# jd-opensource/xllm-service

Measured on NVIDIA H100. Metric: requests/sec tokenize+hash+match @4K-token prompts, higher is better.
Workload: dtype u64

## Files before the change

### xllm_service_b200/csrc/common.cuh

```cuda
#pragma once
#include <cuda_runtime.h>
#include <stdint.h>
#include <stdio.h>

#include <mutex>

#define XLLM_OK 0
#define XLLM_ERR_INVALID_ARG (-1)
#define XLLM_ERR_CUDA (-2)
#define XLLM_ERR_IO (-3)
#define XLLM_ERR_FORMAT (-4)
#define XLLM_ERR_UNSUPPORTED (-5)
#define XLLM_ERR_CAPACITY (-6)
#define XLLM_ERR_NOMEM (-7)

namespace xllm {

void set_last_error(const char* fmt, ...);

#define XLLM_CUDA_TRY(expr)                                                              \
  do {                                                                                   \
    cudaError_t _e = (expr);                                                             \
    if (_e != cudaSuccess) {                                                             \
      ::xllm::set_last_error("%s:%d: %s -> %s", __FILE__, __LINE__, #expr,               \
                             cudaGetErrorString(_e));                                    \
      return XLLM_ERR_CUDA;                                                              \
    }                                                                                    \
  } while (0)

#define XLLM_TRY_RC(expr)          \
  do {                             \
    const int _rc = (expr);        \
    if (_rc != XLLM_OK) return _rc; \
  } while (0)

__device__ __forceinline__ uint32_t smem_u32(const void* p) {
  return static_cast<uint32_t>(__cvta_generic_to_shared(p));
}

__device__ __forceinline__ void cp_async_16(void* smem_dst, const void* gmem_src) {
  asm volatile("cp.async.cg.shared.global [%0], [%1], 16;\n" ::"r"(smem_u32(smem_dst)), "l"(gmem_src)
               : "memory");
}
__device__ __forceinline__ void cp_async_4(void* smem_dst, const void* gmem_src) {
  asm volatile("cp.async.ca.shared.global [%0], [%1], 4;\n" ::"r"(smem_u32(smem_dst)), "l"(gmem_src)
               : "memory");
}
__device__ __forceinline__ void cp_async_commit() { asm volatile("cp.async.commit_group;\n" ::: "memory"); }
template <int N>
__device__ __forceinline__ void cp_async_wait() {
  asm volatile("cp.async.wait_group %0;\n" ::"n"(N) : "memory");
}

struct DeviceOnce {
  static constexpr int kMaxDevices = 64;
  std::once_flag flag[kMaxDevices];
  int n_sm[kMaxDevices] = {0};
  cudaError_t err[kMaxDevices] = {cudaSuccess};
  template <typename F>
  int get(F&& setup, cudaError_t* e, int* device = nullptr) {
    int dev = 0;
    *e = cudaGetDevice(&dev);
    if (*e != cudaSuccess) return 0;
    if (device) *device = dev;
    if (dev < 0 || dev >= kMaxDevices) { *e = cudaErrorInvalidDevice; return 0; }
    std::call_once(flag[dev], [&] {
      int n = 0;
      cudaError_t r = cudaDeviceGetAttribute(&n, cudaDevAttrMultiProcessorCount, dev);
      if (r == cudaSuccess) r = setup();
      n_sm[dev] = n;
      err[dev] = r;
    });
    *e = err[dev];
    return *e == cudaSuccess ? n_sm[dev] : 0;
  }
};

}
```

### xllm_service_b200/csrc/sp_encode.cu

```cuda
#include "sp_encode.cuh"

#include <stdlib.h>
#include <string.h>

#include <type_traits>
#include <vector>

#include "common.cuh"
#include "sp_long_word.cuh"

namespace xllm {

namespace {

constexpr int kNBuf = 2048;
constexpr int kFastWin = 128;
constexpr int kExpWin = 512;
constexpr int kPrefetchFirst = 2;
constexpr int kPrefetchWindows = 2;
constexpr int kLongEnterAt = 1024;
constexpr int kLongFlushAt = 1024;
constexpr int kMaxSym = 16;
constexpr int kCoopMaxSym = 512;
constexpr int kMaxWords = 704;
constexpr uint32_t kFull = 0xffffffffu;
constexpr size_t kWarmSliceBytes = (size_t)kNBuf * 4 + (size_t)kMaxWords * 2;
constexpr uint16_t kNotPre = 0xFFFFu;
constexpr uint32_t kResolvedFlag = 0x40000000u;

template <bool SMALL>
struct PMOps;
template <>
struct PMOps<false> {
  using T = uint2;
  static constexpr uint32_t kNone = kNoPrio;
  static __device__ __forceinline__ T pack(uint2 v) { return v; }
  static __device__ __forceinline__ T none() { return make_uint2(kNoPrio, 0); }
  static __device__ __forceinline__ uint32_t prio(T v) { return v.x; }
  static __device__ __forceinline__ uint32_t merged(T v) { return v.y; }
  static __device__ __forceinline__ uint32_t prio_at(const T* p) { return p->x; }
};
template <>
struct PMOps<true> {
  using T = uint32_t;
  static constexpr uint32_t kNone = 0xFFFFu;
  static __device__ __forceinline__ T pack(uint2 v) { return v.x == kNoPrio ? 0xFFFF0000u : ((v.x << 16) | v.y); }
  static __device__ __forceinline__ T none() { return 0xFFFF0000u; }
  static __device__ __forceinline__ uint32_t prio(T v) { return v >> 16; }
  static __device__ __forceinline__ uint32_t merged(T v) { return v & 0xFFFFu; }
  static __device__ __forceinline__ uint32_t prio_at(const T* p) {
    return reinterpret_cast<const uint16_t*>(p)[1];
  }
};

constexpr int kHfRows = 32;
template <bool SMALL, int ROWS = kMaxSym>
struct WarpSmemT {
  static constexpr int kRows = ROWS;
  static constexpr int kSyms = ROWS * 32 > kCoopMaxSym ? ROWS * 32 : kCoopMaxSym;
  uint32_t S[kSyms];
  typename PMOps<SMALL>::T PM[kSyms];
  uint8_t nbuf[kNBuf];
  uint16_t wstart[kMaxWords];
  uint16_t pend[32];
};
constexpr int kUniMaxMatch = 32;
template <bool SMALL>
struct WarpSmemUniT : WarpSmemT<SMALL> {
  uint32_t mlist[32 * kUniMaxMatch];
};

__device__ __forceinline__ uint32_t hash_pair(uint32_t a, uint32_t b) {
  return (a * 0x9E3779B1u + b) * 0x85EBCA6Bu;
}
__device__ __forceinline__ uint32_t hash_cp(uint32_t cp) {
  uint32_t h = cp * 0x9E3779B1u;
  h ^= h >> 16;
  return h;
}

struct PairProbe {
  uint32_t h;
  uint4 e;
};
__device__ __forceinline__ PairProbe pair_probe_begin(const SpDev& T, uint32_t a, uint32_t b) {
  PairProbe p;
  p.h = hash_pair(a, b) >> T.pair_shift;
  p.e = ((a | b) & kSymUnknownFlag) ? make_uint4(kEmptyKey, 0, 0, 0)
                                    : __ldg(reinterpret_cast<const uint4*>(T.pair_table) + p.h);
  return p;
}
__device__ __forceinline__ uint2 pair_probe_finish(const SpDev& T, uint32_t a, uint32_t b, PairProbe p) {
  for (;;) {
    if (p.e.x == a && p.e.y == b) return make_uint2(p.e.z, p.e.w);
    if (p.e.x == kEmptyKey) return make_uint2(kNoPrio, 0);
    p.h = (p.h + 1) & T.pair_mask;
    p.e = __ldg(reinterpret_cast<const uint4*>(T.pair_table) + p.h);
  }
}
__device__ __forceinline__ uint2 pair_lookup(const SpDev& T, uint32_t a, uint32_t b) {
  return pair_probe_finish(T, a, b, pair_probe_begin(T, a, b));
}

__device__ __forceinline__ uint32_t cp_lookup(const SpDev& T, uint32_t cp) {
  if (cp == 0x2581u) return T.space_sym;
  uint32_t h = hash_cp(cp) & T.cp_mask;
  for (;;) {
    const uint2 e = __ldg(reinterpret_cast<const uint2*>(T.cp_table) + h);
    if (e.x == cp) return e.y;
    if (e.x == kEmptyKey) return kSymUnknownFlag | cp;
    h = (h + 1) & T.cp_mask;
  }
}

__device__ __forceinline__ uint32_t utf8_unit(const uint8_t* p, uint32_t avail, uint8_t b0, bool* valid) {
  *valid = true;
  if (b0 < 0x80) return 1;
  auto trail = [](uint8_t x) { return (x & 0xC0) == 0x80; };
  if (avail >= 2 && (b0 & 0xE0) == 0xC0) {
    const uint8_t b1 = p[1];
    const uint32_t cp = ((b0 & 0x1Fu) << 6) | (b1 & 0x3Fu);
    if (trail(b1) && cp >= 0x80) return 2;
  } else if (avail >= 3 && (b0 & 0xF0) == 0xE0) {
    const uint8_t b1 = p[1], b2 = p[2];
    const uint32_t cp = ((b0 & 0x0Fu) << 12) | ((b1 & 0x3Fu) << 6) | (b2 & 0x3Fu);
    if (trail(b1) && trail(b2) && cp >= 0x800 && !(cp >= 0xD800 && cp < 0xE000)) return 3;
  } else if (avail >= 4 && (b0 & 0xF8) == 0xF0) {
    const uint8_t b1 = p[1], b2 = p[2], b3 = p[3];
    const uint32_t cp = ((b0 & 0x07u) << 18) | ((b1 & 0x3Fu) << 12) | ((b2 & 0x3Fu) << 6) | (b3 & 0x3Fu);
    if (trail(b1) && trail(b2) && trail(b3) && cp >= 0x10000 && cp <= 0x10FFFF) return 4;
  }
  *valid = false;
  return 1;
}

__device__ __forceinline__ uint32_t char_sym(const SpDev& T, const uint8_t* p, uint32_t* adv) {
  const uint32_t b0 = p[0];
  if (b0 < 0x80 || T.byte_mode) {
    *adv = 1;
    return __ldg(T.ascii_sym + b0);
  }
  uint32_t cp, l;
  if (b0 < 0xE0) { l = 2; cp = ((b0 & 0x1F) << 6) | (p[1] & 0x3F); }
  else if (b0 < 0xF0) { l = 3; cp = ((b0 & 0x0F) << 12) | ((p[1] & 0x3Fu) << 6) | (p[2] & 0x3F); }
  else { l = 4; cp = ((b0 & 0x07) << 18) | ((p[1] & 0x3Fu) << 12) | ((p[2] & 0x3Fu) << 6) | (p[3] & 0x3F); }
  *adv = l;
  return cp_lookup(T, cp);
}

__device__ __forceinline__ int sym_ids(const SpDev& T, uint32_t sym, int32_t out[4], bool* unk) {
  uint32_t cp;
  *unk = false;
  if (!(sym & kSymUnknownFlag)) {
    const int32_t e = __ldg(T.emit + sym);
    if (e >= 0) { out[0] = e; return 1; }
    if (e == -2) return 0;
    cp = __ldg(T.virt_cp + (sym - T.n_pieces));
  } else {
    cp = sym & 0x1FFFFFu;
  }
  *unk = true;
  if (!T.byte_fallback) { out[0] = T.unk_id; return 1; }
  uint8_t b[4];
  int n;
  if (cp < 0x80) { b[0] = (uint8_t)cp; n = 1; }
  else if (cp < 0x800) { b[0] = 0xC0 | (cp >> 6); b[1] = 0x80 | (cp & 0x3F); n = 2; }
  else if (cp < 0x10000) { b[0] = 0xE0 | (cp >> 12); b[1] = 0x80 | ((cp >> 6) & 0x3F); b[2] = 0x80 | (cp & 0x3F); n = 3; }
  else { b[0] = 0xF0 | (cp >> 18); b[1] = 0x80 | ((cp >> 12) & 0x3F); b[2] = 0x80 | ((cp >> 6) & 0x3F); b[3] = 0x80 | (cp & 0x3F); n = 4; }
  for (int i = 0; i < n; ++i) out[i] = __ldg(T.byte_id + b[i]);
  return n;
// ... 672 lines not shown
__device__ int unigram_backtrack(SM& sm, const uint8_t* w, int len, int lane);
template <typename SM>
__device__ int unigram_word_slow(const SpDev& T, SM& sm, const uint8_t* w, int len, float* score, int lane);

template <typename SM>
__device__ int unigram_word(const SpDev& T, SM& sm, const uint8_t* w, int len, float* score, int lane) {
  float* best = reinterpret_cast<float*>(sm.S);
  uint32_t* back = reinterpret_cast<uint32_t*>(sm.PM);
  for (int e = lane; e <= len; e += 32) back[e] = 0;
  if (lane == 0) best[0] = *score;
  __syncwarp();
  for (int s0 = 0; s0 < len; s0 += 32) {
    const int s = s0 + lane;
    const bool is_start = s < len && (w[s] & 0xC0) != 0x80;
    int cnt = 0;
    bool overflow = false;
    if (is_start) {
      const uint8_t b0 = w[s];
      int clen = b0 < 0x80 ? 1 : (b0 < 0xE0 ? 2 : (b0 < 0xF0 ? 3 : 4));
      if (clen > len - s) clen = len - s;
      const int max_l = (int)T.max_piece_len < len - s ? (int)T.max_piece_len : len - s;
      uint32_t node = 0;
      bool has_single = false;
      for (int L = 1; L <= max_l; ++L) {
        int32_t piece;
        if (!uni_trie_step(T, node, w[s + L - 1], &node, &piece)) break;
        if (piece >= 0) {
          if (cnt < kUniMaxMatch) sm.mlist[lane * kUniMaxMatch + cnt] = ((uint32_t)L << 24) | (uint32_t)piece;
          else overflow = true;
          ++cnt;
          has_single |= L == clen;
        }
      }
      if (!has_single) {
        if (cnt < kUniMaxMatch) sm.mlist[lane * kUniMaxMatch + cnt] = ((uint32_t)clen << 24) | 0xFFFFFFu;
        else overflow = true;
        ++cnt;
      }
    }
    if (__any_sync(kFull, overflow)) return unigram_word_slow(T, sm, w, len, score, lane);
    __syncwarp();
    uint32_t starts = __ballot_sync(kFull, is_start);
    while (starts) {
      const int b = __ffs(starts) - 1;
      starts &= starts - 1;
      const int sb = s0 + b;
      const int nb_ = __shfl_sync(kFull, cnt, b);
      const float base = best[sb];
      if (lane < nb_) {
        const uint32_t m = sm.mlist[b * kUniMaxMatch + lane];
        const int L = (int)(m >> 24);
        const uint32_t id = m & 0xFFFFFFu;
        const int e = sb + L;
        const double cand = id == 0xFFFFFFu ? (double)(T.unk_score + base)
                                            : (double)__ldg(T.piece_score + id) + (double)base;
        if (back[e] == 0 || cand > (double)best[e]) {
          best[e] = (float)cand;
          back[e] = m;
        }
      }
      __syncwarp();
    }
  }
  const float end_score = best[len];
  __syncwarp();
  const int n = unigram_backtrack(sm, w, len, lane);
  *score = end_score;
  __syncwarp();
  return n;
}

template <typename SM>
__device__ int unigram_backtrack(SM& sm, const uint8_t* w, int len, int lane) {
  const uint32_t* back = reinterpret_cast<const uint32_t*>(sm.PM);
  int n = 0;
  for (int e = len; e > 0; e -= (int)(back[e] >> 24)) ++n;
  __syncwarp();
  if (lane == 0) {
    int k = n;
    for (int e = len; e > 0;) {
      const uint32_t link = back[e];
      const int L = (int)(link >> 24);
      uint32_t sym;
      if ((link & 0xFFFFFFu) != 0xFFFFFFu) {
        sym = kResolvedFlag | (link & 0xFFFFFFu);
      } else {
        const uint8_t* p = w + e - L;
        const uint32_t b0 = p[0];
        uint32_t cp = b0;
        if (L == 2) cp = ((b0 & 0x1F) << 6) | (p[1] & 0x3F);
        else if (L == 3) cp = ((b0 & 0x0F) << 12) | ((p[1] & 0x3Fu) << 6) | (p[2] & 0x3F);
        else if (L == 4) cp = ((b0 & 0x07) << 18) | ((p[1] & 0x3Fu) << 12) | ((p[2] & 0x3Fu) << 6) | (p[3] & 0x3F);
        sym = kSymUnknownFlag | cp;
      }
      sm.S[--k] = sym;
      e -= L;
    }
  }
  __syncwarp();
  return n;
}

template <typename SM>
__device__ int unigram_word_slow(const SpDev& T, SM& sm, const uint8_t* w, int len, float* score, int lane) {
  float* best = reinterpret_cast<float*>(sm.S);
  uint32_t* back = reinterpret_cast<uint32_t*>(sm.PM);
  static_assert(sizeof(sm.S) >= 4 * (kUniMaxWord + 1) && sizeof(sm.PM) >= 4 * (kUniMaxWord + 1), "lattice scratch");
  if (lane == 0) best[0] = *score;
  __syncwarp();
  const int passes = ((int)T.max_piece_len + 31) / 32;
  for (int e = 1; e <= len; ++e) {
    if (e < len && (w[e] & 0xC0) == 0x80) continue;
    int cs = e - 1;
    while (cs > 0 && (w[cs] & 0xC0) == 0x80) --cs;
    const int clen = e - cs;
    float best_f = 0.f;
    uint32_t best_link = 0;
    bool first = true;
    for (int pass = passes - 1; pass >= 0; --pass) {
      const int L = pass * 32 + lane + 1;
      const int s = e - L;
      int32_t id = -1;
      if (L <= (int)T.max_piece_len && s >= 0 && (w[s] & 0xC0) != 0x80) id = hf_vocab_lookup(T, w + s, L);
      const bool unk = id < 0 && L == clen;
      double cand = 0.0;
      if (id >= 0) cand = (double)__ldg(T.piece_score + id) + (double)best[s];
      else if (unk) cand = (double)(T.unk_score + best[s]);
      uint32_t m = __ballot_sync(kFull, id >= 0 || unk);
      while (m) {
        const int src = 31 - __clz(m);
        m &= ~(1u << src);
        const double c = __shfl_sync(kFull, cand, src);
        const int32_t cid = __shfl_sync(kFull, id, src);
        if (first || c > (double)best_f) {
          best_f = (float)c;
          best_link = ((uint32_t)(pass * 32 + src + 1) << 24) | (cid >= 0 ? (uint32_t)cid : 0xFFFFFFu);
          first = false;
        }
      }
    }
    if (lane == 0) { best[e] = best_f; back[e] = best_link; }
    __syncwarp();
  }
  const float end_score = best[len];
  __syncwarp();
  const int n = unigram_backtrack(sm, w, len, lane);
  *score = end_score;
  __syncwarp();
  return n;
}

#ifdef XLLM_EXP_STATS
constexpr int kExpStats = 32;
enum : int { kExpStatTimed = 16, kExpStatCycWindow = 17, kExpStatCycProbe = 18, kExpStatCycEmit = 19 };
__device__ unsigned long long g_exp_stats[kExpStats];
#define EXP_STAT(i) do { if (lane == 0) atomicAdd(&g_exp_stats[i], 1ull); } while (0)
#define EXP_CLOCK(t) (t = clock64())
#else
#define EXP_STAT(i) do { } while (0)
#define EXP_CLOCK(t) do { } while (0)
#endif

struct ExpReq {
  const uint8_t* src;
  uint32_t len;
  int32_t* out;
  int64_t cap;
  int64_t n_out;
  bool P;
  bool S;
  bool U;
};
constexpr int kExpWords = 64;
template <bool SMALL>
struct ExpSmemT {
  uint32_t S[kMaxSym * 32];
  typename PMOps<SMALL>::T PM[kMaxSym * 32];
  uint4 txt[kExpWin / 16 + 1];
  uint16_t ex[2 * (kExpWords + 2)];
};
constexpr int kExpLongWords = 4;
constexpr int kExpLongEvery = 512;
struct ExpResume {
  uint32_t pos;
  uint32_t flags;
  long long n_out;
};

struct ExpLongWord {
  uint32_t end;
  int32_t n_out;
  bool done;
  bool unk;
};

template <bool SMALL, typename SM>
__device__ __noinline__ ExpLongWord express_long_word(const SpDev& T, SM& sm, const uint32_t* base, uint32_t nwords,
                                                      uint32_t vlen, uint32_t v0, bool lead, int32_t* out, int32_t cap,
                                                      int32_t n_out, bool prev_unk, int lane) {
  const ExpLongWord not_done{0u, n_out, false, prev_unk};
  uint32_t end = 0;
  bool found = false;
  for (uint32_t wb = v0 & ~3u; !found; wb += (uint32_t)kFastWin) {
    if (wb - (v0 & ~3u) > (uint32_t)kCoopMaxSym) return not_done;
    const uint32_t i = (wb >> 2) + (uint32_t)lane;
    uint32_t w = i < nwords ? __ldg(base + i) : 0x20202020u;
    const uint32_t b0 = wb + 4u * lane;
    uint32_t sp4 = 0, bad4 = 0;
#pragma unroll
    for (int k = 0; k < 4; ++k) {
      const uint32_t bk = (w >> (8 * k)) & 0xFFu;
      const uint32_t at = b0 + k;
      if (at < v0) continue;
      if (at >= vlen) { sp4 |= 1u << k; continue; }
      if (bk >= 0x80u) { bad4 |= 1u << k; continue; }
      const bool spl = bk == 0x20u || ((T.spacelike_ascii[(bk >> 5) & 3] >> (bk & 31)) & 1u);
      const bool simple = (T.simple_ascii[(bk >> 5) & 3] >> (bk & 31)) & 1u;
      if (spl && (bk != 0x20u || simple)) sp4 |= 1u << k;
      else if (!simple) bad4 |= 1u << k;
    }
    const uint32_t spm = __ballot_sync(kFull, sp4 != 0u), badm = __ballot_sync(kFull, bad4 != 0u);
    if (spm) {
      const int L = __ffs(spm) - 1;
      const uint32_t sL = __shfl_sync(kFull, sp4, L), bL = __shfl_sync(kFull, bad4, L);
      const int k = __ffs(sL) - 1;
      if ((badm & ((1u << L) - 1u)) || (bL & ((1u << k) - 1u))) return not_done;
      end = wb + 4u * L + k;
      found = true;
    } else if (badm) {
      return not_done;
    }
  }
  const int nbytes = (int)(end - v0);
  const int nsym = nbytes + (lead ? 1 : 0);
  if (nbytes < 1 || nsym > kCoopMaxSym) return not_done;
  const uint8_t* bytes = reinterpret_cast<const uint8_t*>(base) + v0;
  __syncwarp();
  if (lead && lane == 0) sm.S[0] = T.space_sym;
  for (int i = lane; i < nbytes; i += 32) sm.S[i + (lead ? 1 : 0)] = __ldg(T.ascii_sym + __ldg(bytes + i));
  __syncwarp();
  const int n = coop_merge<SMALL>(T, sm, nsym, lane);
  for (int b = 0; b < n; b += 32) {
    const int j = b + lane;
    int32_t tmp[4];
    bool unk = false;
    int c = 0;
    if (j < n) c = sym_ids(T, sm.S[j], tmp, &unk);
    if (!T.byte_fallback) {
      const uint32_t um = __ballot_sync(kFull, j < n && unk);
      const bool prev = lane == 0 ? prev_unk : ((um >> (lane - 1)) & 1u);
      if (unk && prev) c = 0;
      const int lastl = (n - b) >= 32 ? 31 : (n - b - 1);
      prev_unk = (um >> lastl) & 1u;
    }
    const int inc = warp_incl_scan(c, lane);
    int32_t o = n_out + (inc - c);
    for (int k = 0; k < c; ++k, ++o)
      if (o < cap) out[o] = tmp[k];
    n_out += __shfl_sync(kFull, inc, 31);
  }
  if (T.byte_fallback) prev_unk = false;
  __syncwarp();
  return ExpLongWord{end, n_out, true, prev_unk};
}

__device__ __forceinline__ uint32_t exp_blank(uint32_t x, int i, int lo, int hi) {
  const int a = min(max(lo - 4 * i, 0), 4), b = min(max(hi - 4 * i, 0), 4);
  const uint32_t below_b = b >= 4 ? 0xFFFFFFFFu : (1u << (8 * b)) - 1u, below_a = a >= 4 ? 0xFFFFFFFFu : (1u << (8 * a)) - 1u;
  const uint32_t keep = below_b & ~below_a;
  return (x & keep) | (0x20202020u & ~keep);
}
__device__ __forceinline__ uint32_t exp_space4(uint32_t x) {
  x ^= 0x20202020u;
  const uint32_t z = ~(((x & 0x7F7F7F7Fu) + 0x7F7F7F7Fu) | x | 0x7F7F7F7Fu);
  return (((z >> 7) * 0x01020408u) >> 24) & 0xFu;
}
__device__ __forceinline__ U128 exp_word_key(const uint4* txt, uint32_t s, int n, bool lead) {
  const uint2* t8 = reinterpret_cast<const uint2*>(txt) + (s >> 3);
  const uint2 u0 = t8[0], u1 = t8[1], u2 = t8[2];
  const bool odd = (s & 4u) != 0u;
  const uint32_t bsh = (s & 3u) * 8u;
  const uint32_t t0 = odd ? u0.y : u0.x, t1 = odd ? u1.x : u0.y, t2 = odd ? u1.y : u1.x, t3 = odd ? u2.x : u1.y,
                 t4 = odd ? u2.y : u2.x;
  unsigned long long lo = (unsigned long long)__funnelshift_r(t0, t1, bsh) | ((unsigned long long)__funnelshift_r(t1, t2, bsh) << 32);
  unsigned long long hi = (unsigned long long)__funnelshift_r(t2, t3, bsh) | ((unsigned long long)__funnelshift_r(t3, t4, bsh) << 32);
  if (n < 8) { lo &= (1ull << (8 * n)) - 1ull; hi = 0ull; }
  else hi &= (1ull << (8 * (n - 8))) - 1ull;
  return U128{(lo << 8) | (unsigned long long)((lead ? 0x80u : 0u) | (uint32_t)n), (hi << 8) | (lo >> 56)};
}
template <bool SMALL>
__device__ __forceinline__ bool exp_probe_finish(MemoRef memo, U128 key, uint32_t slot, U128 k, U128& val) {
  if (k.lo == key.lo && k.hi == key.hi) return MemoIds<SMALL>::valid(val);
  if ((k.lo | k.hi) == 0) return false;
  const uint8_t* e = memo.table + (size_t)(slot ^ 1u) * 32;
  const U128 k2 = ld_b128_cached(e);
  val = ld_b128_cached(e + 16);
  return k2.lo == key.lo && k2.hi == key.hi && MemoIds<SMALL>::valid(val);
}
template <bool SMALL>
__device__ __forceinline__ void exp_store(int32_t* out, U128 val, int cnt, int o, bool c1, bool c2, bool fits,
                                          int32_t cap) {
  if (fits) {
    if (cnt >= 1) out[o] = (int32_t)MemoIds<SMALL>::id(val, 0);
    if (c1 || c2) {
      if (cnt >= 2) out[o + 1] = (int32_t)MemoIds<SMALL>::id(val, 1);
      if (cnt >= 3) out[o + 2] = (int32_t)MemoIds<SMALL>::id(val, 2);
      if (c2) {
#pragma unroll
        for (int q = 3; q < MemoIds<SMALL>::kMax; ++q)
          if (q < cnt) out[o + q] = (int32_t)MemoIds<SMALL>::id(val, q);
      }
    }
  } else {
#pragma unroll
    for (int q = 0; q < MemoIds<SMALL>::kMax; ++q)
      if (q < cnt && o + q < cap) out[o + q] = (int32_t)MemoIds<SMALL>::id(val, q);
  }
}

template <bool SMALL, bool MEMO, typename SM>
__device__ __forceinline__ uint32_t express_run(const SpDev& T, SM& sm, ExpReq& rs, uint32_t pos, int lane,
                                                MemoRef memo, bool* failed) {
  const uint32_t A = (uint32_t)(reinterpret_cast<uintptr_t>(rs.src) & 15u);
  const uint32_t* const base = reinterpret_cast<const uint32_t*>(rs.src - A);
  const uint4* const base16 = reinterpret_cast<const uint4*>(rs.src - A);
  const uint32_t vlen = rs.len + A;
  const uint32_t nwords = (vlen + 3u) >> 2;
  const uint32_t nunits = (vlen + 15u) >> 4;
  bool P = rs.P;
  bool S = rs.S;
  bool U = rs.U;
  int n_long = 0;
  uint16_t* const ex = sm.ex;
  const uint32_t* const ex2 = reinterpret_cast<const uint32_t*>(sm.ex);
  int32_t* const out = rs.out;
  const int32_t cap = rs.cap > 0x7fffffffll ? 0x7fffffff : (int32_t)rs.cap;
  int32_t n_out = (int32_t)rs.n_out;
  const uint32_t lt = (1u << lane) - 1u;
  auto load_window = [&](uint32_t at) {
    const uint32_t i = (at >> 4) + (uint32_t)lane;
    return i < nunits ? __ldg(base16 + i) : make_uint4(0x20202020u, 0x20202020u, 0x20202020u, 0x20202020u);
  };
  uint32_t v = pos + A;
  uint4 w = load_window(v);
  *failed = false;
#ifdef XLLM_EXP_STATS
  unsigned long long t_step = 0, t_vote = 0, t_probe = 0, cyc_window = 0, cyc_probe = 0, cyc_emit = 0, n_timed = 0;
#endif
  for (;;) {
    EXP_CLOCK(t_step);
    const uint32_t skip = v & 15u;
    const uint32_t wb = v - skip;
    const bool at_end = wb + (uint32_t)kExpWin >= vlen;
    if ((skip != 0u && lane == 0) || at_end) {
      const int lo = lane == 0 ? (int)skip : 0;
      const int hi = at_end ? (int)(vlen - wb) - 16 * lane : 16;
      w = make_uint4(exp_blank(w.x, 0, lo, hi), exp_blank(w.y, 1, lo, hi), exp_blank(w.z, 2, lo, hi),
                     exp_blank(w.w, 3, lo, hi));
    }
    {
      bool ok = ((w.x | w.y | w.z | w.w) & 0x80808080u) == 0u;
      bool fast_ok = false;
      if (T.printable_simple)
        fast_ok = (((w.x | 0x80808080u) - 0x20202020u) & ((w.y | 0x80808080u) - 0x20202020u) &
                   ((w.z | 0x80808080u) - 0x20202020u) & ((w.w | 0x80808080u) - 0x20202020u) & 0x80808080u) ==
                      0x80808080u &&
                  (((w.x + 0x01010101u) | (w.y + 0x01010101u) | (w.z + 0x01010101u) | (w.w + 0x01010101u)) &
                   0x80808080u) == 0u;
      if (!__all_sync(kFull, ok && fast_ok)) {
        uint32_t q[4] = {w.x, w.y, w.z, w.w};
#pragma unroll
        for (int k = 0; k < 16; ++k) {
          uint32_t& part = q[k >> 2];
          const uint32_t bk = (part >> (8 * (k & 3))) & 0xFFu;
          const bool spl = (T.spacelike_ascii[(bk >> 5) & 3] >> (bk & 31)) & 1u;
          ok = ok && (spl || ((T.simple_ascii[(bk >> 5) & 3] >> (bk & 31)) & 1u));
          if (spl) part = (part & ~(0xFFu << (8 * (k & 3)))) | (0x20u << (8 * (k & 3)));
        }
        if (!__all_sync(kFull, ok)) { EXP_STAT(4); *failed = true; break; }
        w = make_uint4(q[0], q[1], q[2], q[3]);
      }
    }
    EXP_CLOCK(t_vote);
    const uint32_t ns16 = ~(exp_space4(w.x) | (exp_space4(w.y) << 4) | (exp_space4(w.z) << 8) | (exp_space4(w.w) << 12)) &
                          0xFFFFu;
    sm.txt[lane] = w;
    uint32_t prev_ns = (__shfl_up_sync(kFull, ns16, 1) >> 15) & 1u;
    uint32_t next_ns = __shfl_down_sync(kFull, ns16, 1) & 1u;
    if (lane == 0) prev_ns = 0u;
    if (lane == 31) next_ns = at_end ? 0u : 1u;
    if (!P && !S) {
      if ((__shfl_sync(kFull, ns16, 0) >> skip) & 1u) { EXP_STAT(5); *failed = true; break; }
    }
    const uint32_t st16 = ns16 & ~((ns16 << 1) | prev_ns) & 0xFFFFu;
    const uint32_t en16 = ns16 & ~((ns16 >> 1) | (next_ns << 15)) & 0xFFFFu;
    const uint32_t cs = __popc(st16);
    const uint32_t b0 = __ballot_sync(kFull, cs & 1u), b1 = __ballot_sync(kFull, cs & 2u);
    const uint32_t b2 = __ballot_sync(kFull, cs & 4u), b3 = __ballot_sync(kFull, cs & 8u);
    const uint32_t last_ns = __ballot_sync(kFull, (ns16 & 0x8000u) != 0u) >> 31;
    const int nstart = __popc(b0) + 2 * __popc(b1) + 4 * __popc(b2) + 8 * __popc(b3);
    const int nend = nstart - (int)(at_end ? 0u : last_ns);
    int take = nend < kExpWords ? nend : kExpWords;
    uint32_t cons = at_end ? vlen - wb : (uint32_t)kExpWin - 1u;
    bool S2 = true;
    uint4 w_next = make_uint4(0u, 0u, 0u, 0u);
    auto long_word = [&](uint32_t s0) -> bool {
      ++n_long;
      const bool dense = n_long > kExpLongWords && (uint32_t)n_long * (uint32_t)kExpLongEvery > wb + s0 - A;
      ExpLongWord r{0u, n_out, false, U};
      if (!dense) r = express_long_word<SMALL>(T, sm, base, nwords, vlen, wb + s0, P || (!S && s0 > skip), out, cap,
                                              n_out, U, lane);
      n_out = r.n_out;
      U = r.unk;
      if (!r.done) {
        if (s0 > skip) {
          P = P || !S;
          S = true;
          v = wb + s0;
        }
        *failed = true;
        return false;
      }
      P = false;
      S = false;
      v = r.end;
      if (v >= vlen) return false;
      w = load_window(v);
      return true;
    };
    if (nstart > 0) {
      {
        uint32_t k = __popc(b0 & lt) + 2 * __popc(b1 & lt) + 4 * __popc(b2 & lt) + 8 * __popc(b3 & lt);
        uint32_t e = k - (prev_ns & ns16 & 1u);
        for (uint32_t m = st16; m && k <= (uint32_t)kExpWords; m &= m - 1u, ++k)
          ex[2u * k] = (uint16_t)(16 * lane + __ffs(m) - 1);
        for (uint32_t m = en16; m && e < (uint32_t)kExpWords; m &= m - 1u, ++e)
          ex[2u * e + 1u] = (uint16_t)(16 * lane + __ffs(m) - 1);
      }
      __syncwarp();
      const bool inA = lane < take, inB = lane + 32 < take;
      const uint32_t seA = ex2[inA ? lane : 0], seB = ex2[inB ? lane + 32 : 0];
      const uint32_t sA = seA & 0xFFFFu, sB = seB & 0xFFFFu;
      const int nA = (int)(seA >> 16) - (int)sA + 1, nB = (int)(seB >> 16) - (int)sB + 1;
      const uint32_t lmA = __ballot_sync(kFull, inA && nA > kMemoMaxKeyBytes);
      const uint32_t lmB = __ballot_sync(kFull, inB && nB > kMemoMaxKeyBytes);
      if (lmA) take = __ffs(lmA) - 1;
      else if (lmB) take = 32 + __ffs(lmB) - 1;
      if (take == 0) {
        const uint32_t s0 = ex[0];
        if (!lmA && s0 > skip) {
          cons = s0;
          w_next = load_window(wb + cons);
        } else {
          if (long_word(s0)) { EXP_STAT(6); continue; }
          EXP_STAT(7);
          break;
        }
      } else {
      const bool activeA = lane < take, activeB = lane + 32 < take;
      if (take < nstart) cons = ex[2 * take];
      const bool leadA = lane > 0 || P || (!S && sA > skip);
      const U128 keyA = exp_word_key(sm.txt, sA, nA, leadA), keyB = exp_word_key(sm.txt, sB, nB, true);
      bool hitA = false, hitB = false;
      U128 valA{0ull, 0ull}, valB{0ull, 0ull};
      if constexpr (MEMO) {
        const uint32_t slotA = memo_slot(keyA, memo.mask), slotB = memo_slot(keyB, memo.mask);
        U128 kA{0ull, 0ull}, kB{0ull, 0ull};
        if (activeA) {
          kA = ld_b128_cached(memo.table + (size_t)slotA * 32);
          valA = ld_b128_cached(memo.table + (size_t)slotA * 32 + 16);
        }
        if (activeB) {
          kB = ld_b128_cached(memo.table + (size_t)slotB * 32);
          valB = ld_b128_cached(memo.table + (size_t)slotB * 32 + 16);
        }
        if (activeA) hitA = exp_probe_finish<SMALL>(memo, keyA, slotA, kA, valA);
        if (activeB) hitB = exp_probe_finish<SMALL>(memo, keyB, slotB, kB, valB);
      }
      bool hardA = false, hardB = false;
#pragma unroll 1
      for (int h = 0; h < 2; ++h) {
        if (!(h ? activeB && !hitB : activeA && !hitA)) continue;
        const U128 key = h ? keyB : keyA;
        const unsigned long long lo = (key.lo >> 8) | (key.hi << 56), hi = key.hi >> 8;
        const int n = (int)(key.lo & 0x7Fu);
        int m = 0;
        if (key.lo & 0x80u) { sm.S[lane] = T.space_sym; m = 1; }
        for (int i = 0; i < n; ++i) {
          const uint32_t c = (uint32_t)((i < 8 ? lo >> (8 * i) : hi >> (8 * (i - 8))) & 0xFFull);
          sm.S[(m++) * 32 + lane] = __ldg(T.ascii_sym + c);
        }
        const uint32_t alive = lane_merge<SMALL>(T, sm, m, lane);
        const int k = __popc(alive);
        uint32_t id[8] = {0, 0, 0, 0, 0, 0, 0, 0};
        bool hard = k > MemoIds<SMALL>::kMax;
        int q = 0;
        for (uint32_t mm = alive; mm && !hard; ++q) {
          const int j = __ffs(mm) - 1;
          mm &= mm - 1;
          const uint32_t sym = sm.S[j * 32 + lane];
          int32_t e = -1;
          if (!(sym & kSymUnknownFlag)) e = __ldg(T.emit + sym);
          if (e < 0 || (uint32_t)e >= (SMALL ? (1u << 16) : (1u << 28))) hard = true;
          else id[q] = (uint32_t)e;
        }
        if (!hard) {
          const U128 val = MemoIds<SMALL>::pack(k, id);
          if (h) valB = val;
          else valA = val;
          if constexpr (MEMO) {
            uint32_t slot = memo_slot(key, memo.mask);
            const U128 zero{0ull, 0ull};
#pragma unroll 1
            for (int way = 0; way < 2; ++way, slot ^= 1u) {
              uint8_t* e = memo.table + (size_t)slot * 32;
              const U128 old = cas_b128(e, zero, key);
              if ((old.lo | old.hi) == 0) { st_b128(e + 16, val); break; }
              if (old.lo == key.lo && old.hi == key.hi) break;
            }
          }
        }
        if (h) hardB = hard;
        else hardA = hard;
      }
      {
        const uint32_t hmA = __ballot_sync(kFull, hardA), hmB = __ballot_sync(kFull, hardB);
        EXP_CLOCK(t_probe);
        if (hmA | hmB) {
          const int fh = hmA ? __ffs(hmA) - 1 : 32 + __ffs(hmB) - 1;
          EXP_STAT(8);
          if (fh == 0) {
            if (long_word(ex[0])) continue;
            break;
          }
          take = fh;
          cons = ex[2 * take];
        }
      }
      w_next = load_window(wb + cons);
#ifdef XLLM_EXP_STATS
      { const uint32_t aA = __ballot_sync(kFull, activeA), aB = __ballot_sync(kFull, activeB);
        const uint32_t hA = __ballot_sync(kFull, hitA), hB = __ballot_sync(kFull, hitB);
        if (lane == 0) { atomicAdd(&g_exp_stats[9], (unsigned long long)(__popc(aA) + __popc(aB))); atomicAdd(&g_exp_stats[10], (unsigned long long)(__popc(hA) + __popc(hB))); if ((aA & ~hA) | (aB & ~hB)) atomicAdd(&g_exp_stats[11], 1ull); } }
#endif
      const int cntA = lane < take ? MemoIds<SMALL>::count(valA) : 0;
      const int cntB = lane + 32 < take ? MemoIds<SMALL>::count(valB) : 0;
      const uint32_t a0 = __ballot_sync(kFull, cntA & 1), a1 = __ballot_sync(kFull, cntA & 2), a2 = __ballot_sync(kFull, cntA & 4);
      const uint32_t c0 = __ballot_sync(kFull, cntB & 1), c1 = __ballot_sync(kFull, cntB & 2), c2 = __ballot_sync(kFull, cntB & 4);
      const int totalA = __popc(a0) + 2 * __popc(a1) + 4 * __popc(a2);
      const int totalB = __popc(c0) + 2 * __popc(c1) + 4 * __popc(c2);
      const int oA = n_out + __popc(a0 & lt) + 2 * __popc(a1 & lt) + 4 * __popc(a2 & lt);
      const int oB = n_out + totalA + __popc(c0 & lt) + 2 * __popc(c1 & lt) + 4 * __popc(c2 & lt);
      const bool fits = n_out + totalA + totalB <= cap;
      exp_store<SMALL>(out, valA, cntA, oA, a1 != 0u, a2 != 0u, fits, cap);
      if (c0 | c1 | c2) exp_store<SMALL>(out, valB, cntB, oB, c1 != 0u, c2 != 0u, fits, cap);
      n_out += totalA + totalB;
      U = false;
#ifdef XLLM_EXP_STATS
      { const unsigned long long t = clock64(); cyc_window += t_vote - t_step; cyc_probe += t_probe - t_vote; cyc_emit += t - t_probe; ++n_timed; }
#endif
      if (take == nstart) S2 = !((__shfl_sync(kFull, ns16, (cons - 1u) >> 4) >> ((cons - 1u) & 15u)) & 1u);
      }
    } else {
      w_next = load_window(wb + cons);
    }
    EXP_STAT(1);
    P = S2 && (take > 0 || P || !S);
    S = S2;
    v = wb + cons;
    if (v >= vlen) break;
    w = w_next;
    __syncwarp();
  }
#ifdef XLLM_EXP_STATS
  if (lane == 0) {
    atomicAdd(&g_exp_stats[kExpStatTimed], n_timed);
    atomicAdd(&g_exp_stats[kExpStatCycWindow], cyc_window);
    atomicAdd(&g_exp_stats[kExpStatCycProbe], cyc_probe);
    atomicAdd(&g_exp_stats[kExpStatCycEmit], cyc_emit);
  }
#endif
  rs.P = P;
  rs.S = S;
  rs.U = U;
  rs.n_out = n_out;
  __syncwarp();
  return v - A;
}

constexpr int kExpWarps = 4;
#ifndef XLLM_EXP_MIN_BLOCKS
#define XLLM_EXP_MIN_BLOCKS 6
#endif
template <bool SMALL>
__global__ void __launch_bounds__(kExpWarps * 32, XLLM_EXP_MIN_BLOCKS) sp_express_kernel(
    const uint8_t* __restrict__ text, const int64_t* __restrict__ offsets, int n_req, int32_t* __restrict__ ids,
    int64_t ids_stride, int32_t* __restrict__ n_ids, int32_t* __restrict__ status, const __grid_constant__ SpDev T,
    unsigned int* __restrict__ task_counter, int32_t* __restrict__ legacy_list, unsigned int* __restrict__ legacy_count,
    ExpResume* __restrict__ resume, uint8_t* memo_table, uint32_t memo_mask) {
  const MemoRef memo{memo_table, memo_mask};
  extern __shared__ __align__(16) unsigned char smem_raw[];
  using SM = ExpSmemT<SMALL>;
  SM& sm = reinterpret_cast<SM*>(smem_raw)[threadIdx.x >> 5];
  const int lane = threadIdx.x & 31;
  unsigned long long warp_t0 = 0;
  if (T.warp_ns) asm volatile("mov.u64 %0, %%globaltimer;" : "=l"(warp_t0));
  for (;;) {
    unsigned int r = 0;
    if (lane == 0) r = atomicAdd(task_counter, 1u);
    r = __shfl_sync(kFull, r, 0);
    if (r >= (unsigned)n_req) break;
    ExpReq rq;
    const int64_t beg = offsets[r];
    rq.src = text + beg;
    rq.len = (uint32_t)(offsets[r + 1] - beg);
    rq.out = T.out_start ? ids + T.out_start[r] : ids + (int64_t)r * ids_stride;
    rq.cap = T.out_cap ? (int64_t)T.out_cap[r] : ids_stride;
    rq.n_out = 0;
    rq.P = T.add_dummy_prefix != 0;
    rq.S = true;
    rq.U = false;
    bool failed = false;
    uint32_t pos = 0;
    if (rq.len > 0) pos = express_run<SMALL, true>(T, sm, rq, 0u, lane, memo, &failed);
#ifdef XLLM_EXP_STATS
    if (lane == 0) { atomicAdd(&g_exp_stats[12], (unsigned long long)pos); atomicAdd(&g_exp_stats[13], (unsigned long long)rq.len); atomicAdd(&g_exp_stats[14], failed ? 1ull : 0ull); }
#endif
    if (lane == 0) {
      if (!failed) {
        n_ids[r] = (int32_t)rq.n_out;
        status[r] = rq.n_out > rq.cap ? kEncTruncated : kEncOk;
      } else {
        ExpResume rr;
        rr.pos = pos;
        rr.flags = (rq.P ? 1u : 0u) | (rq.S ? 2u : 0u) | (rq.U ? 4u : 0u);
        rr.n_out = rq.n_out;
        resume[r] = rr;
        legacy_list[atomicAdd(legacy_count, 1u)] = (int32_t)r;
      }
    }
    __syncwarp();
  }
  if (T.warp_ns && lane == 0) {
    unsigned long long t1;
    asm volatile("mov.u64 %0, %%globaltimer;" : "=l"(t1));
    T.warp_ns[blockIdx.x * kExpWarps + (threadIdx.x >> 5)] = t1 - warp_t0;
  }
}

template <typename SM>
__device__ __forceinline__ int gather_chars(const SpDev& T, SM& sm, int ws, int we, bool* overflow, int lane) {
  const uint8_t* nb = sm.nbuf;
  int n = 0;
  bool over = false;
  for (int base = ws; base < we; base += 32) {
    const int p = base + lane;
    const bool lead = p < we && (T.byte_mode || (nb[p] & 0xC0) != 0x80);
    const uint32_t m = __ballot_sync(kFull, lead);
    const int idx = n + __popc(m & ((1u << lane) - 1));
    if (lead) {
      if (idx < kCoopMaxSym) { uint32_t adv; sm.S[idx] = char_sym(T, nb + p, &adv); }
      else over = true;
    }
    n += __popc(m);
  }
  *overflow = __any_sync(kFull, over);
  __syncwarp();
  return n;
}

template <bool SMALL, bool LONG, int MODE, bool MEMO, bool WARM, typename SM>
__device__ bool drain_pass(const SpDev& T, SM& sm, ReqState& rs, bool final, int lane, MemoRef memo) {
  static_assert(!WARM || (MEMO && !LONG && MODE != 2), "the warm-up pre-passes need the memo and the lane path");
  constexpr bool HF = MODE == 1;
  constexpr bool UNI = MODE == 2;
  const uint8_t* nb = sm.nbuf;
  int nlen = rs.nlen;
  if (final && T.remove_extra_ws) {
    while (nlen >= 3 && nb[nlen - 3] == 0xE2 && nb[nlen - 2] == 0x96 && nb[nlen - 1] == 0x81) nlen -= 3;
    if (nlen == 0) { rs.n_out -= rs.trailing_bare; rs.trailing_bare = 0; }
  }
  if (nlen == 0) { rs.nlen = 0; return false; }

  int nwords = 0;
  int hf_tail = 0;
  bool hf_capped = false;
  if constexpr (HF) {
    const HfScan sc = hf_scan(T, sm, nlen, final, lane);
    if (sc.bad) { rs.bad_input = (int8_t)sc.bad; return false; }
    nwords = sc.nwords;
    hf_tail = sc.tail_start;
    hf_capped = sc.capped;
  } else if (!rs.rescan && !(final && nlen != rs.nlen)) {
    nwords = rs.nw;
  } else if (!rs.rescan) {
    nwords = rs.nw;
    while (nwords > 1 && sm.wstart[nwords - 1] >= nlen) --nwords;
  } else {
    for (int base = 0; base < nlen; base += 32) {
      const int p = base + lane;
      bool st = false;
      if (p < nlen) {
        if (p == 0) st = true;
        else if (T.split_mode != 0 && is_space_at(nb, p, nlen)) {
          st = T.split_mode == 1 || !(p >= 3 && is_space_at(nb, p - 3, nlen));
        }
      }
      const uint32_t m = __ballot_sync(kFull, st);
      if (st) sm.wstart[nwords + __popc(m & ((1u << lane) - 1))] = (uint16_t)p;
      nwords += __popc(m);
    }
  }
  __syncwarp();
  if constexpr (!HF) {
    if (lane == 0) sm.wstart[nwords] = (uint16_t)nlen;
    __syncwarp();
  }
  const int complete = HF ? nwords : (final ? nwords : nwords - 1);

  auto word_of = [&](int w, int& ws, int& we, int& nsym, bool& special) {
    ws = we = nsym = 0;
    special = false;
    if constexpr (HF) {
      const uint16_t e = sm.wstart[w];
      ws = e & kHfPosMask;
      we = sm.wstart[w + 1] & kHfPosMask;
      special = (e & kHfSpecialWord) != 0;
      nsym = special ? 1 : we - ws;
    } else {
      ws = sm.wstart[w];
      we = sm.wstart[w + 1];
      if (rs.ascii) nsym = (we - ws) - (nb[ws] == 0xE2 ? 2 : 0);
      else
        for (int p = ws; p < we; ++p) nsym += T.byte_mode || (nb[p] & 0xC0) != 0x80;
// ... 947 lines not shown
```

Measured before the change: 18.94 million.

## Widen express window to 1024 bytes with cp.async loads and multi-pass word probing

Doubles the express-path text window so each lane handles 32 bytes, loading the window into shared memory with cp.async instead of per-lane __ldg registers. Word extraction capacity is doubled, and memo probing now runs in passes of 64 words per iteration. The character-class rewrite gains a cheaper path that only touches control bytes when the table is printable-simple. This is meant to cut the per-window fixed overhead of votes, ballots and loads. It raises shared-memory and register pressure, which may lower occupancy under the existing launch bounds.

```diff
diff --git a/xllm_service_b200/csrc/common.cuh b/xllm_service_b200/csrc/common.cuh
--- a/xllm_service_b200/csrc/common.cuh
+++ b/xllm_service_b200/csrc/common.cuh
@@ -42,6 +42,10 @@
   asm volatile("cp.async.cg.shared.global [%0], [%1], 16;\n" ::"r"(smem_u32(smem_dst)), "l"(gmem_src)
                : "memory");
 }
+__device__ __forceinline__ void cp_async_16_ca(void* smem_dst, const void* gmem_src) {
+  asm volatile("cp.async.ca.shared.global [%0], [%1], 16;\n" ::"r"(smem_u32(smem_dst)), "l"(gmem_src)
+               : "memory");
+}
 __device__ __forceinline__ void cp_async_4(void* smem_dst, const void* gmem_src) {
   asm volatile("cp.async.ca.shared.global [%0], [%1], 4;\n" ::"r"(smem_u32(smem_dst)), "l"(gmem_src)
                : "memory");
diff --git a/xllm_service_b200/csrc/sp_encode.cu b/xllm_service_b200/csrc/sp_encode.cu
--- a/xllm_service_b200/csrc/sp_encode.cu
+++ b/xllm_service_b200/csrc/sp_encode.cu
@@ -1,5 +1,6 @@
 #include "sp_encode.cuh"
 
+#include <assert.h>
 #include <stdlib.h>
 #include <string.h>
 
@@ -15,7 +16,7 @@
 
 constexpr int kNBuf = 2048;
 constexpr int kFastWin = 128;
-constexpr int kExpWin = 512;
+constexpr int kExpWin = 1024;
 constexpr int kPrefetchFirst = 2;
 constexpr int kPrefetchWindows = 2;
 constexpr int kLongEnterAt = 1024;
@@ -994,13 +995,19 @@
 
 #ifdef XLLM_EXP_STATS
 constexpr int kExpStats = 32;
-enum : int { kExpStatTimed = 16, kExpStatCycWindow = 17, kExpStatCycProbe = 18, kExpStatCycEmit = 19 };
+enum : int { kExpStatTimed = 16, kExpStatCycWindow = 17, kExpStatCycProbe0 = 18, kExpStatCycEmit0 = 19,
+             kExpStatCycProbe1 = 20, kExpStatCycEmit1 = 21, kExpStatTimed1 = 22 };
 __device__ unsigned long long g_exp_stats[kExpStats];
 #define EXP_STAT(i) do { if (lane == 0) atomicAdd(&g_exp_stats[i], 1ull); } while (0)
 #define EXP_CLOCK(t) (t = clock64())
 #else
 #define EXP_STAT(i) do { } while (0)
 #define EXP_CLOCK(t) do { } while (0)
+#endif
+#ifdef XLLM_EXP_CHECKS
+#define EXP_CHECK(c) assert(c)
+#else
+#define EXP_CHECK(c) do { } while (0)
 #endif
 
 struct ExpReq {
@@ -1013,13 +1020,17 @@
   bool S;
   bool U;
 };
-constexpr int kExpWords = 64;
+constexpr int kExpPass = 64;
+constexpr int kExpWords = 2 * kExpPass;
 template <bool SMALL>
 struct ExpSmemT {
   uint32_t S[kMaxSym * 32];
   typename PMOps<SMALL>::T PM[kMaxSym * 32];
   uint4 txt[kExpWin / 16 + 1];
   uint16_t ex[2 * (kExpWords + 2)];
+};
+struct ExpWin {
+  uint4 a, b;
 };
 constexpr int kExpLongWords = 4;
 constexpr int kExpLongEvery = 512;
@@ -1117,6 +1128,49 @@
   const uint32_t z = ~(((x & 0x7F7F7F7Fu) + 0x7F7F7F7Fu) | x | 0x7F7F7F7Fu);
   return (((z >> 7) * 0x01020408u) >> 24) & 0xFu;
 }
+__device__ __forceinline__ uint32_t exp_space16(uint4 x) {
+  return exp_space4(x.x) | (exp_space4(x.y) << 4) | (exp_space4(x.z) << 8) | (exp_space4(x.w) << 12);
+}
+__device__ __forceinline__ uint32_t exp_ge20(uint4 x) {
+  return ((x.x | 0x80808080u) - 0x20202020u) & ((x.y | 0x80808080u) - 0x20202020u) &
+         ((x.z | 0x80808080u) - 0x20202020u) & ((x.w | 0x80808080u) - 0x20202020u);
+}
+__device__ __forceinline__ uint32_t exp_eq7f(uint4 x) {
+  return (x.x + 0x01010101u) | (x.y + 0x01010101u) | (x.z + 0x01010101u) | (x.w + 0x01010101u);
+}
+__device__ __forceinline__ bool exp_rewrite(const SpDev& T, uint4& x) {
+  uint32_t q[4] = {x.x, x.y, x.z, x.w};
+  bool ok = true;
+#pragma unroll
+  for (int k = 0; k < 16; ++k) {
+    uint32_t& part = q[k >> 2];
+    const uint32_t bk = (part >> (8 * (k & 3))) & 0xFFu;
+    const bool spl = (T.spacelike_ascii[(bk >> 5) & 3] >> (bk & 31)) & 1u;
+    ok = ok && (spl || ((T.simple_ascii[(bk >> 5) & 3] >> (bk & 31)) & 1u));
+    if (spl) part = (part & ~(0xFFu << (8 * (k & 3)))) | (0x20u << (8 * (k & 3)));
+  }
+  x = make_uint4(q[0], q[1], q[2], q[3]);
+  return ok;
+}
+__device__ __forceinline__ bool exp_rewrite_ctl(const SpDev& T, uint4& x) {
+  uint32_t q[4] = {x.x, x.y, x.z, x.w};
+  bool ok = true;
+#pragma unroll
+  for (int i = 0; i < 4; ++i) {
+    const uint32_t u = q[i];
+    uint32_t m = (~((u | 0x80808080u) - 0x20202020u) | (u + 0x01010101u)) & 0x80808080u;
+    while (m) {
+      const int sh = __ffs(m) - 8;
+      m &= m - 1u;
+      const uint32_t bk = (u >> sh) & 0xFFu;
+      const bool spl = (T.spacelike_ascii[(bk >> 5) & 3] >> (bk & 31)) & 1u;
+      ok = ok && (spl || ((T.simple_ascii[(bk >> 5) & 3] >> (bk & 31)) & 1u));
+      if (spl) q[i] = (q[i] & ~(0xFFu << sh)) | (0x20u << sh);
+    }
+  }
+  x = make_uint4(q[0], q[1], q[2], q[3]);
+  return ok;
+}
 __device__ __forceinline__ U128 exp_word_key(const uint4* txt, uint32_t s, int n, bool lead) {
   const uint2* t8 = reinterpret_cast<const uint2*>(txt) + (s >> 3);
   const uint2 u0 = t8[0], u1 = t8[1], u2 = t8[2];
@@ -1180,72 +1234,70 @@
   int32_t n_out = (int32_t)rs.n_out;
   const uint32_t lt = (1u << lane) - 1u;
   auto load_window = [&](uint32_t at) {
-    const uint32_t i = (at >> 4) + (uint32_t)lane;
-    return i < nunits ? __ldg(base16 + i) : make_uint4(0x20202020u, 0x20202020u, 0x20202020u, 0x20202020u);
+    const uint32_t i = (at >> 4) + 2u * (uint32_t)lane;
+    if (i < nunits) cp_async_16_ca(&sm.txt[2 * lane], base16 + i);
+    if (i + 1u < nunits) cp_async_16_ca(&sm.txt[2 * lane + 1], base16 + i + 1u);
+    cp_async_commit();
   };
   uint32_t v = pos + A;
-  uint4 w = load_window(v);
+  load_window(v);
   *failed = false;
 #ifdef XLLM_EXP_STATS
-  unsigned long long t_step = 0, t_vote = 0, t_probe = 0, cyc_window = 0, cyc_probe = 0, cyc_emit = 0, n_timed = 0;
+  unsigned long long t_step = 0, t_pass = 0, t_probe = 0, cyc_window = 0, cyc_probe[2] = {0, 0}, cyc_emit[2] = {0, 0},
+                     n_timed = 0, n_timed1 = 0;
 #endif
   for (;;) {
     EXP_CLOCK(t_step);
     const uint32_t skip = v & 15u;
     const uint32_t wb = v - skip;
     const bool at_end = wb + (uint32_t)kExpWin >= vlen;
+    cp_async_wait<0>();
+    ExpWin w{sm.txt[2 * lane], sm.txt[2 * lane + 1]};
     if ((skip != 0u && lane == 0) || at_end) {
       const int lo = lane == 0 ? (int)skip : 0;
-      const int hi = at_end ? (int)(vlen - wb) - 16 * lane : 16;
-      w = make_uint4(exp_blank(w.x, 0, lo, hi), exp_blank(w.y, 1, lo, hi), exp_blank(w.z, 2, lo, hi),
-                     exp_blank(w.w, 3, lo, hi));
+      const int hi = at_end ? (int)(vlen - wb) - 32 * lane : 32;
+      w.a = make_uint4(exp_blank(w.a.x, 0, lo, hi), exp_blank(w.a.y, 1, lo, hi), exp_blank(w.a.z, 2, lo, hi),
+                       exp_blank(w.a.w, 3, lo, hi));
+      w.b = make_uint4(exp_blank(w.b.x, 4, lo, hi), exp_blank(w.b.y, 5, lo, hi), exp_blank(w.b.z, 6, lo, hi),
+                       exp_blank(w.b.w, 7, lo, hi));
     }
     {
-      bool ok = ((w.x | w.y | w.z | w.w) & 0x80808080u) == 0u;
+      bool ok = ((w.a.x | w.a.y | w.a.z | w.a.w | w.b.x | w.b.y | w.b.z | w.b.w) & 0x80808080u) == 0u;
       bool fast_ok = false;
       if (T.printable_simple)
-        fast_ok = (((w.x | 0x80808080u) - 0x20202020u) & ((w.y | 0x80808080u) - 0x20202020u) &
-                   ((w.z | 0x80808080u) - 0x20202020u) & ((w.w | 0x80808080u) - 0x20202020u) & 0x80808080u) ==
-                      0x80808080u &&
-                  (((w.x + 0x01010101u) | (w.y + 0x01010101u) | (w.z + 0x01010101u) | (w.w + 0x01010101u)) &
-                   0x80808080u) == 0u;
+        fast_ok = ((exp_ge20(w.a) & exp_ge20(w.b) & 0x80808080u) == 0x80808080u) &&
+                  (((exp_eq7f(w.a) | exp_eq7f(w.b)) & 0x80808080u) == 0u);
       if (!__all_sync(kFull, ok && fast_ok)) {
-        uint32_t q[4] = {w.x, w.y, w.z, w.w};
-#pragma unroll
-        for (int k = 0; k < 16; ++k) {
-          uint32_t& part = q[k >> 2];
-          const uint32_t bk = (part >> (8 * (k & 3))) & 0xFFu;
-          const bool spl = (T.spacelike_ascii[(bk >> 5) & 3] >> (bk & 31)) & 1u;
-          ok = ok && (spl || ((T.simple_ascii[(bk >> 5) & 3] >> (bk & 31)) & 1u));
-          if (spl) part = (part & ~(0xFFu << (8 * (k & 3)))) | (0x20u << (8 * (k & 3)));
+        if (ok) {
+          const bool oa = T.printable_simple ? exp_rewrite_ctl(T, w.a) : exp_rewrite(T, w.a);
+          const bool ob = T.printable_simple ? exp_rewrite_ctl(T, w.b) : exp_rewrite(T, w.b);
+          ok = oa && ob;
         }
         if (!__all_sync(kFull, ok)) { EXP_STAT(4); *failed = true; break; }
-        w = make_uint4(q[0], q[1], q[2], q[3]);
-      }
-    }
-    EXP_CLOCK(t_vote);
-    const uint32_t ns16 = ~(exp_space4(w.x) | (exp_space4(w.y) << 4) | (exp_space4(w.z) << 8) | (exp_space4(w.w) << 12)) &
-                          0xFFFFu;
-    sm.txt[lane] = w;
-    uint32_t prev_ns = (__shfl_up_sync(kFull, ns16, 1) >> 15) & 1u;
-    uint32_t next_ns = __shfl_down_sync(kFull, ns16, 1) & 1u;
+      }
+    }
+    const uint32_t ns = ~(exp_space16(w.a) | (exp_space16(w.b) << 16));
+    sm.txt[2 * lane] = w.a;
+    sm.txt[2 * lane + 1] = w.b;
+    uint32_t prev_ns = __shfl_up_sync(kFull, ns, 1) >> 31;
+    uint32_t next_ns = __shfl_down_sync(kFull, ns, 1) & 1u;
     if (lane == 0) prev_ns = 0u;
     if (lane == 31) next_ns = at_end ? 0u : 1u;
     if (!P && !S) {
-      if ((__shfl_sync(kFull, ns16, 0) >> skip) & 1u) { EXP_STAT(5); *failed = true; break; }
-    }
-    const uint32_t st16 = ns16 & ~((ns16 << 1) | prev_ns) & 0xFFFFu;
-    const uint32_t en16 = ns16 & ~((ns16 >> 1) | (next_ns << 15)) & 0xFFFFu;
-    const uint32_t cs = __popc(st16);
+      if ((__shfl_sync(kFull, ns, 0) >> skip) & 1u) { EXP_STAT(5); *failed = true; break; }
+    }
+    const uint32_t st = ns & ~((ns << 1) | prev_ns);
+    const uint32_t en = ns & ~((ns >> 1) | (next_ns << 31));
+    const uint32_t cs = __popc(st);
     const uint32_t b0 = __ballot_sync(kFull, cs & 1u), b1 = __ballot_sync(kFull, cs & 2u);
     const uint32_t b2 = __ballot_sync(kFull, cs & 4u), b3 = __ballot_sync(kFull, cs & 8u);
-    const uint32_t last_ns = __ballot_sync(kFull, (ns16 & 0x8000u) != 0u) >> 31;
-    const int nstart = __popc(b0) + 2 * __popc(b1) + 4 * __popc(b2) + 8 * __popc(b3);
+    const uint32_t b4 = __ballot_sync(kFull, cs & 16u);
+    const uint32_t last_ns = __ballot_sync(kFull, (ns >> 31) != 0u) >> 31;
+    const int nstart = __popc(b0) + 2 * __popc(b1) + 4 * __popc(b2) + 8 * __popc(b3) + 16 * __popc(b4);
     const int nend = nstart - (int)(at_end ? 0u : last_ns);
     int take = nend < kExpWords ? nend : kExpWords;
     uint32_t cons = at_end ? vlen - wb : (uint32_t)kExpWin - 1u;
     bool S2 = true;
-    uint4 w_next = make_uint4(0u, 0u, 0u, 0u);
     auto long_word = [&](uint32_t s0) -> bool {
       ++n_long;
       const bool dense = n_long > kExpLongWords && (uint32_t)n_long * (uint32_t)kExpLongEvery > wb + s0 - A;
@@ -1267,41 +1319,62 @@
       S = false;
       v = r.end;
       if (v >= vlen) return false;
-      w = load_window(v);
+      load_window(v);
       return true;
     };
     if (nstart > 0) {
       {
-        uint32_t k = __popc(b0 & lt) + 2 * __popc(b1 & lt) + 4 * __popc(b2 & lt) + 8 * __popc(b3 & lt);
-        uint32_t e = k - (prev_ns & ns16 & 1u);
-        for (uint32_t m = st16; m && k <= (uint32_t)kExpWords; m &= m - 1u, ++k)
-          ex[2u * k] = (uint16_t)(16 * lane + __ffs(m) - 1);
-        for (uint32_t m = en16; m && e < (uint32_t)kExpWords; m &= m - 1u, ++e)
-          ex[2u * e + 1u] = (uint16_t)(16 * lane + __ffs(m) - 1);
+        uint32_t k = __popc(b0 & lt) + 2 * __popc(b1 & lt) + 4 * __popc(b2 & lt) + 8 * __popc(b3 & lt) +
+                     16 * __popc(b4 & lt);
+        uint32_t e = k - (prev_ns & ns & 1u);
+        for (uint32_t m = st; m && k <= (uint32_t)kExpWords; m &= m - 1u, ++k) {
+          EXP_CHECK(2u * k < (uint32_t)(2 * (kExpWords + 2)));
+          ex[2u * k] = (uint16_t)(32 * lane + __ffs(m) - 1);
+        }
+        for (uint32_t m = en; m && e < (uint32_t)kExpWords; m &= m - 1u, ++e) {
+          EXP_CHECK(2u * e + 1u < (uint32_t)(2 * (kExpWords + 2)));
+          ex[2u * e + 1u] = (uint16_t)(32 * lane + __ffs(m) - 1);
+        }
       }
       __syncwarp();
-      const bool inA = lane < take, inB = lane + 32 < take;
-      const uint32_t seA = ex2[inA ? lane : 0], seB = ex2[inB ? lane + 32 : 0];
-      const uint32_t sA = seA & 0xFFFFu, sB = seB & 0xFFFFu;
-      const int nA = (int)(seA >> 16) - (int)sA + 1, nB = (int)(seB >> 16) - (int)sB + 1;
-      const uint32_t lmA = __ballot_sync(kFull, inA && nA > kMemoMaxKeyBytes);
-      const uint32_t lmB = __ballot_sync(kFull, inB && nB > kMemoMaxKeyBytes);
-      if (lmA) take = __ffs(lmA) - 1;
-      else if (lmB) take = 32 + __ffs(lmB) - 1;
+      const int nfull = take;
+#pragma unroll
+      for (int q = kExpWords / 32 - 1; q >= 0; --q) {
+        const int j = 32 * q + lane;
+        const bool in = j < nfull;
+        const uint32_t se = ex2[in ? j : 0];
+        const uint32_t lm = __ballot_sync(kFull, in && (int)(se >> 16) - (int)(se & 0xFFFFu) + 1 > kMemoMaxKeyBytes);
+        if (lm) take = 32 * q + __ffs(lm) - 1;
+      }
       if (take == 0) {
         const uint32_t s0 = ex[0];
-        if (!lmA && s0 > skip) {
+        if (nfull == 0 && s0 > skip) {
           cons = s0;
-          w_next = load_window(wb + cons);
+          load_window(wb + cons);
         } else {
           if (long_word(s0)) { EXP_STAT(6); continue; }
           EXP_STAT(7);
           break;
         }
       } else {
-      const bool activeA = lane < take, activeB = lane + 32 < take;
       if (take < nstart) cons = ex[2 * take];
-      const bool leadA = lane > 0 || P || (!S && sA > skip);
+      int pb = 0;
+      bool hand = false;
+#ifdef XLLM_EXP_STATS
+      ++n_timed;
+      cyc_window += clock64() - t_step;
+#endif
+#pragma unroll 1
+      for (;;) {
+      EXP_CLOCK(t_pass);
+      const int jA = pb + lane, jB = pb + lane + 32;
+      const bool activeA = jA < take, activeB = jB < take;
+      EXP_CHECK(jB < kExpWords);
+      const uint32_t seA = ex2[activeA ? jA : 0], seB = ex2[activeB ? jB : 0];
+      const uint32_t sA = seA & 0xFFFFu, sB = seB & 0xFFFFu;
+      const int nA = (int)(seA >> 16) - (int)sA + 1, nB = (int)(seB >> 16) - (int)sB + 1;
+      EXP_CHECK(sA < (uint32_t)kExpWin && sB < (uint32_t)kExpWin);
+      const bool leadA = jA > 0 || P || (!S && sA > skip);
       const U128 keyA = exp_word_key(sm.txt, sA, nA, leadA), keyB = exp_word_key(sm.txt, sB, nB, true);
       bool hitA = false, hitB = false;
       U128 valA{0ull, 0ull}, valB{0ull, 0ull};
@@ -1369,24 +1442,22 @@
         const uint32_t hmA = __ballot_sync(kFull, hardA), hmB = __ballot_sync(kFull, hardB);
         EXP_CLOCK(t_probe);
         if (hmA | hmB) {
-          const int fh = hmA ? __ffs(hmA) - 1 : 32 + __ffs(hmB) - 1;
+          const int fh = pb + (hmA ? __ffs(hmA) - 1 : 32 + __ffs(hmB) - 1);
           EXP_STAT(8);
-          if (fh == 0) {
-            if (long_word(ex[0])) continue;
-            break;
-          }
+          if (fh == 0) { hand = true; break; }
           take = fh;
           cons = ex[2 * take];
         }
       }
-      w_next = load_window(wb + cons);
+      const bool last = pb + kExpPass >= take;
+      if (last) load_window(wb + cons);
 #ifdef XLLM_EXP_STATS
       { const uint32_t aA = __ballot_sync(kFull, activeA), aB = __ballot_sync(kFull, activeB);
         const uint32_t hA = __ballot_sync(kFull, hitA), hB = __ballot_sync(kFull, hitB);
         if (lane == 0) { atomicAdd(&g_exp_stats[9], (unsigned long long)(__popc(aA) + __popc(aB))); atomicAdd(&g_exp_stats[10], (unsigned long long)(__popc(hA) + __popc(hB))); if ((aA & ~hA) | (aB & ~hB)) atomicAdd(&g_exp_stats[11], 1ull); } }
 #endif
-      const int cntA = lane < take ? MemoIds<SMALL>::count(valA) : 0;
-      const int cntB = lane + 32 < take ? MemoIds<SMALL>::count(valB) : 0;
+      const int cntA = jA < take ? MemoIds<SMALL>::count(valA) : 0;
+      const int cntB = jB < take ? MemoIds<SMALL>::count(valB) : 0;
       const uint32_t a0 = __ballot_sync(kFull, cntA & 1), a1 = __ballot_sync(kFull, cntA & 2), a2 = __ballot_sync(kFull, cntA & 4);
       const uint32_t c0 = __ballot_sync(kFull, cntB & 1), c1 = __ballot_sync(kFull, cntB & 2), c2 = __ballot_sync(kFull, cntB & 4);
       const int totalA = __popc(a0) + 2 * __popc(a1) + 4 * __popc(a2);
@@ -1394,34 +1465,45 @@
       const int oA = n_out + __popc(a0 & lt) + 2 * __popc(a1 & lt) + 4 * __popc(a2 & lt);
       const int oB = n_out + totalA + __popc(c0 & lt) + 2 * __popc(c1 & lt) + 4 * __popc(c2 & lt);
       const bool fits = n_out + totalA + totalB <= cap;
+      EXP_CHECK(!fits || (oA + cntA <= cap && oB + cntB <= cap));
       exp_store<SMALL>(out, valA, cntA, oA, a1 != 0u, a2 != 0u, fits, cap);
       if (c0 | c1 | c2) exp_store<SMALL>(out, valB, cntB, oB, c1 != 0u, c2 != 0u, fits, cap);
       n_out += totalA + totalB;
       U = false;
 #ifdef XLLM_EXP_STATS
-      { const unsigned long long t = clock64(); cyc_window += t_vote - t_step; cyc_probe += t_probe - t_vote; cyc_emit += t - t_probe; ++n_timed; }
+      { const unsigned long long t = clock64(); const int p = pb ? 1 : 0; cyc_probe[p] += t_probe - t_pass; cyc_emit[p] += t - t_probe; n_timed1 += p; }
 #endif
-      if (take == nstart) S2 = !((__shfl_sync(kFull, ns16, (cons - 1u) >> 4) >> ((cons - 1u) & 15u)) & 1u);
+      if (last) break;
+      pb += kExpPass;
+      }
+      if (hand) {
+        if (long_word(ex[0])) continue;
+        break;
+      }
+      if (take == nstart) S2 = !((__shfl_sync(kFull, ns, (cons - 1u) >> 5) >> ((cons - 1u) & 31u)) & 1u);
       }
     } else {
-      w_next = load_window(wb + cons);
+      load_window(wb + cons);
     }
     EXP_STAT(1);
     P = S2 && (take > 0 || P || !S);
     S = S2;
     v = wb + cons;
     if (v >= vlen) break;
-    w = w_next;
     __syncwarp();
   }
 #ifdef XLLM_EXP_STATS
   if (lane == 0) {
     atomicAdd(&g_exp_stats[kExpStatTimed], n_timed);
+    atomicAdd(&g_exp_stats[kExpStatTimed1], n_timed1);
     atomicAdd(&g_exp_stats[kExpStatCycWindow], cyc_window);
-    atomicAdd(&g_exp_stats[kExpStatCycProbe], cyc_probe);
-    atomicAdd(&g_exp_stats[kExpStatCycEmit], cyc_emit);
+    atomicAdd(&g_exp_stats[kExpStatCycProbe0], cyc_probe[0]);
+    atomicAdd(&g_exp_stats[kExpStatCycEmit0], cyc_emit[0]);
+    atomicAdd(&g_exp_stats[kExpStatCycProbe1], cyc_probe[1]);
+    atomicAdd(&g_exp_stats[kExpStatCycEmit1], cyc_emit[1]);
   }
 #endif
+  cp_async_wait<0>();
   rs.P = P;
   rs.S = S;
   rs.U = U;
```

New measurement: 19.55 million, median of 6. 3.2% higher.
